# luo-yining/CFDBench

Measured on NVIDIA H100. Metric: fno_rollout_steps_per_sec, higher is better.
Workload: dtype bf16

## Files before the change

cfdbench_b200/csrc/fno_dft_fwd_tc.cu:

```cuda
#include "fno_common.cuh"
#include "tc_common.cuh"
#include "tc_tma.cuh"
#include <math.h>
#include <stddef.h>
#include <string.h>

namespace fno {

constexpr int kTdWG = 2;
constexpr int kTdThreads = 128 * kTdWG;
constexpr int kTdPlanes = 2;
constexpr uint32_t kTdPlaneBytes = kHW * 2;
constexpr uint32_t kTdXBytes = kTdPlanes * kTdPlaneBytes;
constexpr int kTdNA = 72;
constexpr uint32_t kTdLboTA = (kTdNA / 8) * 128;
constexpr uint32_t kTdTABytes = 8 * kTdLboTA;
constexpr int kTdK2 = 128, kTdN2 = kTdPlanes * kM2;
constexpr int kTdM2 = 64;
constexpr uint32_t kTdLboA2 = (kTdM2 / 8) * 128;
constexpr uint32_t kTdLboB2 = (kTdN2 / 8) * 128;
constexpr int kTdA2Floats = kTdM2 * kTdK2;

struct TdSmem {
  alignas(1024) unsigned char x[kTdWG][2][kTdXBytes];
  alignas(128) unsigned char ta[kTdTABytes];
  alignas(128) float a2_hi[kTdA2Floats];
  alignas(128) float a2_lo[kTdA2Floats];
  alignas(128) float b2[kTdWG][2][kTdN2 * kTdK2];
  alignas(8) uint64_t x_full[kTdWG][2];
};

__global__ void __launch_bounds__(kTdThreads, 1)
    dft_fwd_tc_kernel(const __grid_constant__ CUtensorMap x_map, float2* __restrict__ xm,
                      const unsigned char* __restrict__ ta_tab, const float* __restrict__ a2_tab, int n_units, int batch,
                      float s0, float s1) {
  extern __shared__ __align__(1024) unsigned char smem_raw[];
  TdSmem& sm = *reinterpret_cast<TdSmem*>(smem_raw);
  if ((smem_u32(smem_raw) & 1023u) != 0) __trap();
  const int tid = threadIdx.x, lane = tid & 31;
  const int wg = tc::warp_index_uniform() >> 2, wq = (tid >> 5) & 3, t = tid & 127, q = lane & 3;
  const int first = blockIdx.x * kTdWG + wg, stride = gridDim.x * kTdWG;
  const int n_mine = first < n_units ? (n_units - first + stride - 1) / stride : 0;

  if (tid == 0) {
    for (int i = 0; i < kTdWG; ++i) { mbar_init(&sm.x_full[i][0], 1); mbar_init(&sm.x_full[i][1], 1); }
    fence_mbar_init();
  }
  for (int e = tid; e < static_cast<int>(kTdTABytes / 16); e += kTdThreads)
    reinterpret_cast<uint4*>(sm.ta)[e] = __ldg(reinterpret_cast<const uint4*>(ta_tab) + e);
  for (int e = tid; e < kTdA2Floats / 4; e += kTdThreads) {
    reinterpret_cast<float4*>(sm.a2_hi)[e] = __ldg(reinterpret_cast<const float4*>(a2_tab) + e);
    reinterpret_cast<float4*>(sm.a2_lo)[e] = __ldg(reinterpret_cast<const float4*>(a2_tab + kTdA2Floats) + e);
  }
  tc::fence_proxy_async_smem();
  __syncthreads();
  pdl_wait();
  pdl_launch_dependents();

  auto load = [&](int i) {
    mbar_expect_tx(&sm.x_full[wg][i & 1], kTdXBytes);
    tma_load_2d(sm.x[wg][i & 1], &x_map, 0, (first + i * stride) * (kTdPlanes * kH), &sm.x_full[wg][i & 1]);
  };
  if (t == 0) {
    if (n_mine > 0) load(0);
    if (n_mine > 1) load(1);
  }
  const int m0 = 16 * wq + (lane >> 2);
  const uint32_t ta_s = tc::smem_addr(sm.ta);
  float* b2_hi = sm.b2[wg][0];
  float* b2_lo = sm.b2[wg][1];
#pragma unroll 1
  for (int i = 0; i < n_mine; ++i) {
    const int s = i & 1;
    mbar_wait(&sm.x_full[wg][s], (i >> 1) & 1);
    float ga[kTdPlanes][36];
    tc::wg_fence();
    const uint32_t x_s = tc::smem_addr(sm.x[wg][s]);
#pragma unroll
    for (int p = 0; p < kTdPlanes; ++p)
#pragma unroll
      for (int ks = 0; ks < kW / 16; ++ks)
        tc::wg_bf16_ss_n72(ga[p], tc::make_smem_desc_sw128(x_s + p * kTdPlaneBytes + ks * 32),
                           tc::make_smem_desc(ta_s + ks * 2 * kTdLboTA, kTdLboTA, 128), ks ? 1u : 0u);
    tc::wg_commit();
    tc::wg_wait<0>();
    tc::wg_fence_acc(ga[0]);
    tc::wg_fence_acc(ga[1]);
    if (t == 0 && i + 2 < n_mine) load(i + 2);
#pragma unroll
    for (int p = 0; p < kTdPlanes; ++p)
#pragma unroll
      for (int g3 = 0; g3 < 3; ++g3)
#pragma unroll
        for (int hh = 0; hh < 2; ++hh)
#pragma unroll
          for (int ri = 0; ri < 2; ++ri) {
            const int c = 4 * (3 * g3) + 2 * hh + ri;
            const float gsum = (ga[p][c + 8] + ga[p][c + 4]) + ga[p][c];
            float hi, lo;
            tc::split_tf32(gsum, hi, lo);
            const uint32_t off = tc::kmajor_offset(2 * (4 * g3 + q) + p, 64 * ri + m0 + 8 * hh, kTdN2) / 4;
            b2_hi[off] = hi;
            b2_lo[off] = lo;
          }
    tc::fence_proxy_async_smem();
    tc::named_barrier(1 + wg, 128);
    float fb[12];
    tc::wg_fence();
    {
      const uint32_t a_s[3] = {tc::smem_addr(sm.a2_hi), tc::smem_addr(sm.a2_lo), tc::smem_addr(sm.a2_hi)};
      const uint32_t b_s[3] = {tc::smem_addr(b2_hi), tc::smem_addr(b2_hi), tc::smem_addr(b2_lo)};
#pragma unroll
      for (int pass = 0; pass < 3; ++pass)
#pragma unroll
        for (int ks = 0; ks < kTdK2 / 8; ++ks)
          tc::wg_tf32_ss_n24(fb, tc::make_smem_desc(a_s[pass] + ks * 2 * kTdLboA2, kTdLboA2, 128),
                             tc::make_smem_desc(b_s[pass] + ks * 2 * kTdLboB2, kTdLboB2, 128), (pass | ks) ? 1u : 0u);
    }
    tc::wg_commit();
    tc::wg_wait<0>();
    tc::wg_fence_acc(fb);
    const int part = (lane >> 2) & 1;
    const int plane0 = (first + i * stride) * kTdPlanes;
    const int b = plane0 / kC, c0 = plane0 % kC;
#pragma unroll
    for (int j = 0; j < 3; ++j)
#pragma unroll
      for (int hh = 0; hh < 2; ++hh) {
        const int qq = 4 * j + q, m2 = m0 + 8 * hh, kxi = m2 >> 1;
        const float sc = qq == 0 ? s0 : s1;
        const float v0 = fb[4 * j + 2 * hh] * sc, v1 = fb[4 * j + 2 * hh + 1] * sc;
        const float got = __shfl_xor_sync(0xffffffffu, part ? v0 : v1, 4);
        if (m2 < 2 * kKX) {
          float2* dst = xm + (static_cast<size_t>(kxi * kM2 + qq) * batch + b) * kC + c0 + part;
          *dst = part ? make_float2(got, v1) : make_float2(v0, got);
        }
      }
  }
}

static uint16_t td_bf16_bits(double v) {
  float f = static_cast<float>(v);
  uint32_t u;
  memcpy(&u, &f, 4);
  const uint32_t r = u + 0x7fffu + ((u >> 16) & 1u);
  return static_cast<uint16_t>(r >> 16);
}
static double td_bf16_value(uint16_t b) {
  const uint32_t u = static_cast<uint32_t>(b) << 16;
  float f;
  memcpy(&f, &u, 4);
  return static_cast<double>(f);
}
static float td_round_tf32(double v) {
  float f = static_cast<float>(v);
  uint32_t u;
  memcpy(&u, &f, 4);
  u = (u + 0x1000u) & 0xffffe000u;
  memcpy(&f, &u, 4);
  return f;
}

struct TdTables {
  unsigned char* ta = nullptr;
  float* a2 = nullptr;
  int n_sm = 0;
  bool configured = false;
};
static TdTables g_td[64];

static cudaError_t td_ensure(int dev, cudaStream_t stream) {
  TdTables& t = g_td[dev];
  if (t.configured) return cudaSuccess;
  static unsigned char h_ta[kTdTABytes];
  static float h_a2[2 * kTdA2Floats];
  memset(h_ta, 0, sizeof(h_ta));
  memset(h_a2, 0, sizeof(h_a2));
  const double two_pi = 2.0 * 3.14159265358979323846;
  for (int q = 0; q < kM2; ++q)
    for (int ri = 0; ri < 2; ++ri)
      for (int w = 0; w < 64; ++w) {
        const double ang = two_pi * ((q * w) % 64) / 64.0;
        double rest = ri ? -sin(ang) : cos(ang);
        for (int t3 = 0; t3 < 3; ++t3) {
          const int row = 8 * (3 * (q >> 2) + t3) + 2 * (q & 3) + ri;
          const size_t off = static_cast<size_t>(w >> 3) * kTdLboTA + (row >> 3) * 128 + (row & 7) * 16 + (w & 7) * 2;
          const uint16_t bits = td_bf16_bits(rest);
          memcpy(h_ta + off, &bits, 2);
          rest -= td_bf16_value(bits);
        }
      }
  for (int kxi = 0; kxi < kKX; ++kxi) {
    const int kx = kxi < kM1 ? kxi : kxi + (kH - kKX);
    for (int part = 0; part < 2; ++part)
      for (int ri = 0; ri < 2; ++ri)
        for (int h = 0; h < 64; ++h) {
          const double ang = two_pi * ((kx * h) % 64) / 64.0;
          const double c = cos(ang), s = sin(ang);
          const double val = part == 0 ? (ri == 0 ? c : s) : (ri == 0 ? -s : c);
          const uint32_t off = tc::kmajor_offset(2 * kxi + part, ri * 64 + h, kTdM2) / 4;
          const float hi = td_round_tf32(val);
          h_a2[off] = hi;
          h_a2[kTdA2Floats + off] = td_round_tf32(val - static_cast<double>(hi));
        }
  }
  cudaError_t e = cudaMalloc(&t.ta, sizeof(h_ta));
  if (e != cudaSuccess) return e;
  e = cudaMalloc(&t.a2, sizeof(h_a2));
  if (e != cudaSuccess) return e;
  e = cudaMemcpyAsync(t.ta, h_ta, sizeof(h_ta), cudaMemcpyHostToDevice, stream);
  if (e != cudaSuccess) return e;
  e = cudaMemcpyAsync(t.a2, h_a2, sizeof(h_a2), cudaMemcpyHostToDevice, stream);
  if (e != cudaSuccess) return e;
  e = cudaStreamSynchronize(stream);
  if (e != cudaSuccess) return e;
  e = cudaFuncSetAttribute(dft_fwd_tc_kernel, cudaFuncAttributeMaxDynamicSharedMemorySize, (int)sizeof(TdSmem));
  if (e != cudaSuccess) return e;
  e = cudaDeviceGetAttribute(&t.n_sm, cudaDevAttrMultiProcessorCount, dev);
  if (e != cudaSuccess) return e;
  t.configured = true;
  return cudaSuccess;
}

void dft_fwd_tc_release(int dev) {
  if (dev < 0 || dev >= 64) return;
  TdTables& t = g_td[dev];
  if (t.ta) cudaFree(t.ta);
  if (t.a2) cudaFree(t.a2);
  t = TdTables();
}

cudaError_t launch_dft_fwd_tc(const void* x, void* xm, int batch, float s0, float s1, cudaStream_t stream) {
  int dev = 0;
  cudaError_t e = cudaGetDevice(&dev);
  if (e != cudaSuccess) return e;
  if (dev < 0 || dev >= 64) return cudaErrorInvalidDevice;
  e = td_ensure(dev, stream);
  if (e != cudaSuccess) return e;
  if ((reinterpret_cast<uintptr_t>(x) & 15) || (reinterpret_cast<uintptr_t>(xm) & 15)) return cudaErrorMisalignedAddress;
  CUtensorMap map;
  e = make_tma_map_2d(&map, CU_TENSOR_MAP_DATA_TYPE_BFLOAT16, 2, x, kW, static_cast<uint64_t>(batch) * kC * kH, kW,
                      kTdPlanes * kH);
  if (e != cudaSuccess) return e;
  const int n_units = batch * kC / kTdPlanes;
  const int want = (n_units + kTdWG - 1) / kTdWG;
  const int grid = want < g_td[dev].n_sm ? want : g_td[dev].n_sm;
  return launch_chained(dft_fwd_tc_kernel, dim3(grid), dim3(kTdThreads), sizeof(TdSmem), stream, map,
                        static_cast<float2*>(xm), static_cast<const unsigned char*>(g_td[dev].ta),
                        static_cast<const float*>(g_td[dev].a2), n_units, batch, s0, s1);
}

}
```

cfdbench_b200/csrc/tc_common.cuh:

```cuda
#pragma once
#include <cuda_runtime.h>
#include <stdint.h>

namespace fno {
namespace tc {

__device__ __forceinline__ uint32_t smem_addr(const void* p) {
  return static_cast<uint32_t>(__cvta_generic_to_shared(p));
}

__device__ __forceinline__ int warp_index_uniform() {
  return __shfl_sync(0xffffffffu, static_cast<int>(threadIdx.x >> 5), 0);
}

__device__ __forceinline__ void named_barrier(int id, int count) {
  asm volatile("bar.sync %0, %1;" ::"r"(id), "r"(count) : "memory");
}

__device__ __forceinline__ void fence_proxy_async_smem() {
  asm volatile("fence.proxy.async.shared::cta;" ::: "memory");
}

__device__ __forceinline__ uint64_t make_smem_desc(uint32_t saddr, uint32_t lbo_bytes, uint32_t sbo_bytes) {
  uint64_t d = 0;
  d |= static_cast<uint64_t>((saddr & 0x3FFFFu) >> 4);
  d |= static_cast<uint64_t>((lbo_bytes >> 4) & 0x3FFFu) << 16;
  d |= static_cast<uint64_t>((sbo_bytes >> 4) & 0x3FFFu) << 32;
  return d;
}
__device__ __forceinline__ uint64_t make_smem_desc_sw128(uint32_t saddr) {
  return make_smem_desc(saddr, 16, 1024) | (static_cast<uint64_t>(1) << 62);
}
__device__ __forceinline__ uint64_t make_smem_desc_sw128_mn(uint32_t saddr) {
  return make_smem_desc(saddr, 16, 1024) | (static_cast<uint64_t>(1) << 62);
}

__device__ __forceinline__ void wg_fence() { asm volatile("wgmma.fence.sync.aligned;" ::: "memory"); }
__device__ __forceinline__ void wg_commit() { asm volatile("wgmma.commit_group.sync.aligned;" ::: "memory"); }
template <int kPending>
__device__ __forceinline__ void wg_wait() { asm volatile("wgmma.wait_group.sync.aligned %0;" ::"n"(kPending) : "memory"); }
template <int N>
__device__ __forceinline__ void wg_fence_acc(float (&d)[N]) {
#pragma unroll
  for (int i = 0; i < N; ++i) asm volatile("" : "+f"(d[i])::"memory");
}

__device__ __forceinline__ void wg_tf32_ss_n24(float* d, uint64_t a, uint64_t b, uint32_t acc) {
  asm volatile(
      "{\n.reg .pred p;\nsetp.ne.b32 p, %14, 0;\n"
      "wgmma.mma_async.sync.aligned.m64n24k8.f32.tf32.tf32 {%0, %1, %2, %3, %4, %5, %6, %7, %8, %9, %10, %11}, %12, %13, p, 1, 1;\n}\n"
      : "+f"(d[0]), "+f"(d[1]), "+f"(d[2]), "+f"(d[3]), "+f"(d[4]), "+f"(d[5]), "+f"(d[6]), "+f"(d[7]), "+f"(d[8]), "+f"(d[9]), "+f"(d[10]), "+f"(d[11])
      : "l"(a), "l"(b), "r"(acc)
      : "memory");
}
__device__ __forceinline__ void wg_tf32_ss_n32(float* d, uint64_t a, uint64_t b, uint32_t acc) {
  asm volatile(
      "{\n.reg .pred p;\nsetp.ne.b32 p, %18, 0;\n"
      "wgmma.mma_async.sync.aligned.m64n32k8.f32.tf32.tf32 {%0, %1, %2, %3, %4, %5, %6, %7, %8, %9, %10, %11, %12, %13, %14, %15}, %16, %17, p, 1, 1;\n}\n"
      : "+f"(d[0]), "+f"(d[1]), "+f"(d[2]), "+f"(d[3]), "+f"(d[4]), "+f"(d[5]), "+f"(d[6]), "+f"(d[7]), "+f"(d[8]), "+f"(d[9]), "+f"(d[10]), "+f"(d[11]), "+f"(d[12]), "+f"(d[13]), "+f"(d[14]), "+f"(d[15])
      : "l"(a), "l"(b), "r"(acc)
      : "memory");
}
__device__ __forceinline__ void wg_tf32_ss_n128(float* d, uint64_t a, uint64_t b, uint32_t acc) {
  asm volatile(
      "{\n.reg .pred p;\nsetp.ne.b32 p, %66, 0;\n"
      "wgmma.mma_async.sync.aligned.m64n128k8.f32.tf32.tf32 {%0, %1, %2, %3, %4, %5, %6, %7, %8, %9, %10, %11, %12, %13, %14, %15, %16, %17, %18, %19, %20, %21, %22, %23, %24, %25, %26, %27, %28, %29, %30, %31, %32, %33, %34, %35, %36, %37, %38, %39, %40, %41, %42, %43, %44, %45, %46, %47, %48, %49, %50, %51, %52, %53, %54, %55, %56, %57, %58, %59, %60, %61, %62, %63}, %64, %65, p, 1, 1;\n}\n"
      : "+f"(d[0]), "+f"(d[1]), "+f"(d[2]), "+f"(d[3]), "+f"(d[4]), "+f"(d[5]), "+f"(d[6]), "+f"(d[7]), "+f"(d[8]), "+f"(d[9]), "+f"(d[10]), "+f"(d[11]), "+f"(d[12]), "+f"(d[13]), "+f"(d[14]), "+f"(d[15]), "+f"(d[16]), "+f"(d[17]), "+f"(d[18]), "+f"(d[19]), "+f"(d[20]), "+f"(d[21]), "+f"(d[22]), "+f"(d[23]), "+f"(d[24]), "+f"(d[25]), "+f"(d[26]), "+f"(d[27]), "+f"(d[28]), "+f"(d[29]), "+f"(d[30]), "+f"(d[31]), "+f"(d[32]), "+f"(d[33]), "+f"(d[34]), "+f"(d[35]), "+f"(d[36]), "+f"(d[37]), "+f"(d[38]), "+f"(d[39]), "+f"(d[40]), "+f"(d[41]), "+f"(d[42]), "+f"(d[43]), "+f"(d[44]), "+f"(d[45]), "+f"(d[46]), "+f"(d[47]), "+f"(d[48]), "+f"(d[49]), "+f"(d[50]), "+f"(d[51]), "+f"(d[52]), "+f"(d[53]), "+f"(d[54]), "+f"(d[55]), "+f"(d[56]), "+f"(d[57]), "+f"(d[58]), "+f"(d[59]), "+f"(d[60]), "+f"(d[61]), "+f"(d[62]), "+f"(d[63])
      : "l"(a), "l"(b), "r"(acc)
      : "memory");
}
__device__ __forceinline__ void wg_bf16_ss_n72(float* d, uint64_t a, uint64_t b, uint32_t acc) {
  asm volatile(
      "{\n.reg .pred p;\nsetp.ne.b32 p, %38, 0;\n"
      "wgmma.mma_async.sync.aligned.m64n72k16.f32.bf16.bf16 {%0, %1, %2, %3, %4, %5, %6, %7, %8, %9, %10, %11, %12, %13, %14, %15, %16, %17, %18, %19, %20, %21, %22, %23, %24, %25, %26, %27, %28, %29, %30, %31, %32, %33, %34, %35}, %36, %37, p, 1, 1, 0, 0;\n}\n"
      : "+f"(d[0]), "+f"(d[1]), "+f"(d[2]), "+f"(d[3]), "+f"(d[4]), "+f"(d[5]), "+f"(d[6]), "+f"(d[7]), "+f"(d[8]), "+f"(d[9]), "+f"(d[10]), "+f"(d[11]), "+f"(d[12]), "+f"(d[13]), "+f"(d[14]), "+f"(d[15]), "+f"(d[16]), "+f"(d[17]), "+f"(d[18]), "+f"(d[19]), "+f"(d[20]), "+f"(d[21]), "+f"(d[22]), "+f"(d[23]), "+f"(d[24]), "+f"(d[25]), "+f"(d[26]), "+f"(d[27]), "+f"(d[28]), "+f"(d[29]), "+f"(d[30]), "+f"(d[31]), "+f"(d[32]), "+f"(d[33]), "+f"(d[34]), "+f"(d[35])
      : "l"(a), "l"(b), "r"(acc)
      : "memory");
}
__device__ __forceinline__ void wg_bf16_ss_n32_mn_a(float* d, uint64_t a, uint64_t b, uint32_t acc) {
  asm volatile(
      "{\n.reg .pred p;\nsetp.ne.b32 p, %18, 0;\n"
      "wgmma.mma_async.sync.aligned.m64n32k16.f32.bf16.bf16 {%0, %1, %2, %3, %4, %5, %6, %7, %8, %9, %10, %11, %12, %13, %14, %15}, %16, %17, p, 1, 1, 1, 0;\n}\n"
      : "+f"(d[0]), "+f"(d[1]), "+f"(d[2]), "+f"(d[3]), "+f"(d[4]), "+f"(d[5]), "+f"(d[6]), "+f"(d[7]), "+f"(d[8]), "+f"(d[9]), "+f"(d[10]), "+f"(d[11]), "+f"(d[12]), "+f"(d[13]), "+f"(d[14]), "+f"(d[15])
      : "l"(a), "l"(b), "r"(acc)
      : "memory");
}
__device__ __forceinline__ void wg_tf32_rs_n32(float* d, const uint32_t* a, uint64_t b, uint32_t acc) {
  asm volatile(
      "{\n.reg .pred p;\nsetp.ne.b32 p, %21, 0;\n"
      "wgmma.mma_async.sync.aligned.m64n32k8.f32.tf32.tf32 {%0, %1, %2, %3, %4, %5, %6, %7, %8, %9, %10, %11, %12, %13, %14, %15}, {%16, %17, %18, %19}, %20, p, 1, 1;\n}\n"
      : "+f"(d[0]), "+f"(d[1]), "+f"(d[2]), "+f"(d[3]), "+f"(d[4]), "+f"(d[5]), "+f"(d[6]), "+f"(d[7]), "+f"(d[8]), "+f"(d[9]), "+f"(d[10]), "+f"(d[11]), "+f"(d[12]), "+f"(d[13]), "+f"(d[14]), "+f"(d[15])
      : "r"(a[0]), "r"(a[1]), "r"(a[2]), "r"(a[3]), "l"(b), "r"(acc)
      : "memory");
}
__device__ __forceinline__ void wg_tf32_rs_n64(float* d, const uint32_t* a, uint64_t b, uint32_t acc) {
  asm volatile(
      "{\n.reg .pred p;\nsetp.ne.b32 p, %37, 0;\n"
      "wgmma.mma_async.sync.aligned.m64n64k8.f32.tf32.tf32 {%0, %1, %2, %3, %4, %5, %6, %7, %8, %9, %10, %11, %12, %13, %14, %15, %16, %17, %18, %19, %20, %21, %22, %23, %24, %25, %26, %27, %28, %29, %30, %31}, {%32, %33, %34, %35}, %36, p, 1, 1;\n}\n"
      : "+f"(d[0]), "+f"(d[1]), "+f"(d[2]), "+f"(d[3]), "+f"(d[4]), "+f"(d[5]), "+f"(d[6]), "+f"(d[7]), "+f"(d[8]), "+f"(d[9]), "+f"(d[10]), "+f"(d[11]), "+f"(d[12]), "+f"(d[13]), "+f"(d[14]), "+f"(d[15]), "+f"(d[16]), "+f"(d[17]), "+f"(d[18]), "+f"(d[19]), "+f"(d[20]), "+f"(d[21]), "+f"(d[22]), "+f"(d[23]), "+f"(d[24]), "+f"(d[25]), "+f"(d[26]), "+f"(d[27]), "+f"(d[28]), "+f"(d[29]), "+f"(d[30]), "+f"(d[31])
      : "r"(a[0]), "r"(a[1]), "r"(a[2]), "r"(a[3]), "l"(b), "r"(acc)
      : "memory");
}

__host__ __device__ constexpr uint32_t kmajor_offset(int row, int k, int rows) {
  return static_cast<uint32_t>(((k >> 2) * (rows >> 3) + (row >> 3)) * 128 + (row & 7) * 16 + (k & 3) * 4);
}
__device__ __forceinline__ float round_tf32(float x) {
  return __uint_as_float((__float_as_uint(x) + 0x1000u) & 0xffffe000u);
}
__device__ __forceinline__ void split_tf32(float x, float& hi, float& lo) {
  hi = round_tf32(x);
  lo = round_tf32(x - hi);
}

}
}
```

Baseline: 1202.

## Restructure forward DFT stage B to batch eight planes per unit with register-A TF32 wgmma

Each work unit grows from two to eight planes, loaded as four two-plane TMA boxes through a three-slot pipeline. The second (H-direction) DFT stage is transposed so the plane/mode dimension becomes M (three full m64 tiles) and the twiddle table becomes the shared-memory B operand. Intermediates are staged in a swizzled fp32 buffer and split into hi/lo TF32 in registers for RS wgmma at n48. This is meant to replace the narrow n24 stage-B MMAs, which were padded and under-used, with fuller tiles, and to cut the shuffle-based output writes. In exchange it needs more shared memory, more registers per thread for the A fragments, and a grid sized to balance units per pipe.

```diff
diff --git a/cfdbench_b200/csrc/fno_dft_fwd_tc.cu b/cfdbench_b200/csrc/fno_dft_fwd_tc.cu
--- a/cfdbench_b200/csrc/fno_dft_fwd_tc.cu
+++ b/cfdbench_b200/csrc/fno_dft_fwd_tc.cu
@@ -9,133 +9,153 @@
 
 constexpr int kTdWG = 2;
 constexpr int kTdThreads = 128 * kTdWG;
-constexpr int kTdPlanes = 2;
+constexpr int kTdPlanes = 8;
+constexpr int kTdBoxPlanes = 2;
+constexpr int kTdBoxes = kTdPlanes / kTdBoxPlanes;
+constexpr int kTdSlots = 3;
 constexpr uint32_t kTdPlaneBytes = kHW * 2;
-constexpr uint32_t kTdXBytes = kTdPlanes * kTdPlaneBytes;
+constexpr uint32_t kTdBoxBytes = kTdBoxPlanes * kTdPlaneBytes;
 constexpr int kTdNA = 72;
 constexpr uint32_t kTdLboTA = (kTdNA / 8) * 128;
 constexpr uint32_t kTdTABytes = 8 * kTdLboTA;
-constexpr int kTdK2 = 128, kTdN2 = kTdPlanes * kM2;
-constexpr int kTdM2 = 64;
-constexpr uint32_t kTdLboA2 = (kTdM2 / 8) * 128;
-constexpr uint32_t kTdLboB2 = (kTdN2 / 8) * 128;
-constexpr int kTdA2Floats = kTdM2 * kTdK2;
+constexpr int kTdM2 = kM2 * 2 * kTdPlanes;
+constexpr int kTdN2 = 2 * kKX;
+constexpr int kTdK2 = kH;
+constexpr uint32_t kTdLboT = (kTdN2 / 8) * 128;
+constexpr int kTdTFloats = kTdN2 * kTdK2;
+static_assert(kTdM2 == 3 * 64, "stage B is three full m64 tiles");
+
+__host__ __device__ constexpr int td_slot(int n) { return n % kTdSlots; }
+__host__ __device__ constexpr uint32_t td_parity(int n) { return static_cast<uint32_t>(n / kTdSlots) & 1u; }
+__host__ __device__ constexpr int td_box_row(int unit, int box) { return (unit * kTdPlanes + box * kTdBoxPlanes) * kH; }
+__host__ __device__ constexpr int td_unit(int first, int stride, int i) { return first + i * stride; }
+__host__ __device__ constexpr int td_units_of(int first, int stride, int n_units) {
+  return first < n_units ? (n_units - first + stride - 1) / stride : 0;
+}
+__host__ __device__ constexpr int td_g_index(int m, int h) {
+  return m * kTdK2 + (h ^ (((m & 7) << 2) ^ (((m >> 4) & 3) << 3)));
+}
 
 struct TdSmem {
-  alignas(1024) unsigned char x[kTdWG][2][kTdXBytes];
+  alignas(1024) unsigned char x[kTdWG][kTdSlots][kTdBoxBytes];
   alignas(128) unsigned char ta[kTdTABytes];
-  alignas(128) float a2_hi[kTdA2Floats];
-  alignas(128) float a2_lo[kTdA2Floats];
-  alignas(128) float b2[kTdWG][2][kTdN2 * kTdK2];
-  alignas(8) uint64_t x_full[kTdWG][2];
+  alignas(128) float t_hi[kTdTFloats];
+  alignas(128) float t_lo[kTdTFloats];
+  alignas(128) float g[kTdWG][kTdM2 * kTdK2];
+  alignas(8) uint64_t x_full[kTdWG][kTdSlots];
 };
+static_assert(sizeof(TdSmem) <= 232448, "dft_fwd_tc_kernel exceeds the sm_90 opt-in shared memory");
 
 __global__ void __launch_bounds__(kTdThreads, 1)
     dft_fwd_tc_kernel(const __grid_constant__ CUtensorMap x_map, float2* __restrict__ xm,
-                      const unsigned char* __restrict__ ta_tab, const float* __restrict__ a2_tab, int n_units, int batch,
+                      const unsigned char* __restrict__ ta_tab, const float* __restrict__ t_tab, int n_units, int batch,
                       float s0, float s1) {
   extern __shared__ __align__(1024) unsigned char smem_raw[];
   TdSmem& sm = *reinterpret_cast<TdSmem*>(smem_raw);
   if ((smem_u32(smem_raw) & 1023u) != 0) __trap();
   const int tid = threadIdx.x, lane = tid & 31;
-  const int wg = tc::warp_index_uniform() >> 2, wq = (tid >> 5) & 3, t = tid & 127, q = lane & 3;
+  const int wg = tc::warp_index_uniform() >> 2, wq = (tid >> 5) & 3, t = tid & 127, q = lane & 3, lr = lane >> 2;
   const int first = blockIdx.x * kTdWG + wg, stride = gridDim.x * kTdWG;
-  const int n_mine = first < n_units ? (n_units - first + stride - 1) / stride : 0;
+  const int n_mine = td_units_of(first, stride, n_units);
+  const int n_fills = n_mine * kTdBoxes;
 
   if (tid == 0) {
-    for (int i = 0; i < kTdWG; ++i) { mbar_init(&sm.x_full[i][0], 1); mbar_init(&sm.x_full[i][1], 1); }
+    for (int i = 0; i < kTdWG; ++i)
+      for (int s = 0; s < kTdSlots; ++s) mbar_init(&sm.x_full[i][s], 1);
     fence_mbar_init();
   }
   for (int e = tid; e < static_cast<int>(kTdTABytes / 16); e += kTdThreads)
     reinterpret_cast<uint4*>(sm.ta)[e] = __ldg(reinterpret_cast<const uint4*>(ta_tab) + e);
-  for (int e = tid; e < kTdA2Floats / 4; e += kTdThreads) {
-    reinterpret_cast<float4*>(sm.a2_hi)[e] = __ldg(reinterpret_cast<const float4*>(a2_tab) + e);
-    reinterpret_cast<float4*>(sm.a2_lo)[e] = __ldg(reinterpret_cast<const float4*>(a2_tab + kTdA2Floats) + e);
+  for (int e = tid; e < kTdTFloats / 4; e += kTdThreads) {
+    reinterpret_cast<float4*>(sm.t_hi)[e] = __ldg(reinterpret_cast<const float4*>(t_tab) + e);
+    reinterpret_cast<float4*>(sm.t_lo)[e] = __ldg(reinterpret_cast<const float4*>(t_tab + kTdTFloats) + e);
   }
   tc::fence_proxy_async_smem();
   __syncthreads();
   pdl_wait();
   pdl_launch_dependents();
 
-  auto load = [&](int i) {
-    mbar_expect_tx(&sm.x_full[wg][i & 1], kTdXBytes);
-    tma_load_2d(sm.x[wg][i & 1], &x_map, 0, (first + i * stride) * (kTdPlanes * kH), &sm.x_full[wg][i & 1]);
+  auto load = [&](int n) {
+    uint64_t* bar = &sm.x_full[wg][td_slot(n)];
+    mbar_expect_tx(bar, kTdBoxBytes);
+    tma_load_2d(sm.x[wg][td_slot(n)], &x_map, 0, td_box_row(td_unit(first, stride, n / kTdBoxes), n % kTdBoxes), bar);
   };
-  if (t == 0) {
-    if (n_mine > 0) load(0);
-    if (n_mine > 1) load(1);
-  }
-  const int m0 = 16 * wq + (lane >> 2);
+  if (t == 0)
+    for (int n = 0; n < kTdSlots && n < n_fills; ++n) load(n);
+  const int m0 = 16 * wq + lr;
   const uint32_t ta_s = tc::smem_addr(sm.ta);
-  float* b2_hi = sm.b2[wg][0];
-  float* b2_lo = sm.b2[wg][1];
+  float* g = sm.g[wg];
 #pragma unroll 1
   for (int i = 0; i < n_mine; ++i) {
-    const int s = i & 1;
-    mbar_wait(&sm.x_full[wg][s], (i >> 1) & 1);
-    float ga[kTdPlanes][36];
-    tc::wg_fence();
-    const uint32_t x_s = tc::smem_addr(sm.x[wg][s]);
-#pragma unroll
-    for (int p = 0; p < kTdPlanes; ++p)
-#pragma unroll
-      for (int ks = 0; ks < kW / 16; ++ks)
-        tc::wg_bf16_ss_n72(ga[p], tc::make_smem_desc_sw128(x_s + p * kTdPlaneBytes + ks * 32),
-                           tc::make_smem_desc(ta_s + ks * 2 * kTdLboTA, kTdLboTA, 128), ks ? 1u : 0u);
-    tc::wg_commit();
-    tc::wg_wait<0>();
-    tc::wg_fence_acc(ga[0]);
-    tc::wg_fence_acc(ga[1]);
-    if (t == 0 && i + 2 < n_mine) load(i + 2);
-#pragma unroll
-    for (int p = 0; p < kTdPlanes; ++p)
-#pragma unroll
-      for (int g3 = 0; g3 < 3; ++g3)
-#pragma unroll
-        for (int hh = 0; hh < 2; ++hh)
-#pragma unroll
-          for (int ri = 0; ri < 2; ++ri) {
-            const int c = 4 * (3 * g3) + 2 * hh + ri;
-            const float gsum = (ga[p][c + 8] + ga[p][c + 4]) + ga[p][c];
-            float hi, lo;
-            tc::split_tf32(gsum, hi, lo);
-            const uint32_t off = tc::kmajor_offset(2 * (4 * g3 + q) + p, 64 * ri + m0 + 8 * hh, kTdN2) / 4;
-            b2_hi[off] = hi;
-            b2_lo[off] = lo;
-          }
-    tc::fence_proxy_async_smem();
+#pragma unroll 1
+    for (int k = 0; k < kTdBoxes; ++k) {
+      const int n = i * kTdBoxes + k;
+      mbar_wait(&sm.x_full[wg][td_slot(n)], td_parity(n));
+      float ga[kTdBoxPlanes][36];
+      tc::wg_fence();
+      const uint32_t x_s = tc::smem_addr(sm.x[wg][td_slot(n)]);
+#pragma unroll
+      for (int p = 0; p < kTdBoxPlanes; ++p)
+#pragma unroll
+        for (int ks = 0; ks < kW / 16; ++ks)
+          tc::wg_bf16_ss_n72(ga[p], tc::make_smem_desc_sw128(x_s + p * kTdPlaneBytes + ks * 32),
+                             tc::make_smem_desc(ta_s + ks * 2 * kTdLboTA, kTdLboTA, 128), ks ? 1u : 0u);
+      tc::wg_commit();
+      tc::wg_wait<0>();
+      tc::wg_fence_acc(ga[0]);
+      tc::wg_fence_acc(ga[1]);
+      if (t == 0 && n + kTdSlots < n_fills) load(n + kTdSlots);
+      if (k == 0) tc::named_barrier(1 + wg, 128);
+#pragma unroll
+      for (int p = 0; p < kTdBoxPlanes; ++p)
+#pragma unroll
+        for (int g3 = 0; g3 < 3; ++g3)
+#pragma unroll
+          for (int hh = 0; hh < 2; ++hh)
+#pragma unroll
+            for (int ri = 0; ri < 2; ++ri) {
+              const int c = 4 * (3 * g3) + 2 * hh + ri;
+              g[td_g_index(16 * (4 * g3 + q) + 8 * ri + kTdBoxPlanes * k + p, m0 + 8 * hh)] =
+                  (ga[p][c + 8] + ga[p][c + 4]) + ga[p][c];
+            }
+    }
     tc::named_barrier(1 + wg, 128);
-    float fb[12];
-    tc::wg_fence();
-    {
-      const uint32_t a_s[3] = {tc::smem_addr(sm.a2_hi), tc::smem_addr(sm.a2_lo), tc::smem_addr(sm.a2_hi)};
-      const uint32_t b_s[3] = {tc::smem_addr(b2_hi), tc::smem_addr(b2_hi), tc::smem_addr(b2_lo)};
-#pragma unroll
-      for (int pass = 0; pass < 3; ++pass)
+    const int unit = td_unit(first, stride, i);
+    const int b = unit * kTdPlanes / kC, c0 = unit * kTdPlanes % kC;
+#pragma unroll 1
+    for (int tile = 0; tile < kTdM2 / 64; ++tile) {
+      uint32_t a_hi[kTdK2 / 8][4], a_lo[kTdK2 / 8][4];
+#pragma unroll
+      for (int ks = 0; ks < kTdK2 / 8; ++ks)
+#pragma unroll
+        for (int r = 0; r < 4; ++r) {
+          float hi, lo;
+          tc::split_tf32(g[td_g_index(64 * tile + m0 + 8 * (r & 1), 8 * ks + q + 4 * (r >> 1))], hi, lo);
+          a_hi[ks][r] = __float_as_uint(hi);
+          a_lo[ks][r] = __float_as_uint(lo);
+        }
+      float d[24];
+      tc::wg_fence();
+#pragma unroll
+      for (int pass = 0; pass < 3; ++pass) {
+        const uint32_t tb = tc::smem_addr(pass == 1 ? sm.t_lo : sm.t_hi);
 #pragma unroll
         for (int ks = 0; ks < kTdK2 / 8; ++ks)
-          tc::wg_tf32_ss_n24(fb, tc::make_smem_desc(a_s[pass] + ks * 2 * kTdLboA2, kTdLboA2, 128),
-                             tc::make_smem_desc(b_s[pass] + ks * 2 * kTdLboB2, kTdLboB2, 128), (pass | ks) ? 1u : 0u);
+          tc::wg_tf32_rs_n48(d, pass == 2 ? a_lo[ks] : a_hi[ks], tc::make_smem_desc(tb + ks * 2 * kTdLboT, kTdLboT, 128),
+                             (pass | ks) ? 1u : 0u);
+      }
+      tc::wg_commit();
+      tc::wg_wait<0>();
+      tc::wg_fence_acc(d);
+      const int qq = 4 * tile + wq;
+      const float sc = qq == 0 ? s0 : s1;
+#pragma unroll
+      for (int j = 0; j < kTdN2 / 8; ++j) {
+        const int kxi = 4 * j + q;
+        const float re = (d[4 * j + 0] + d[4 * j + 3]) * sc, im = (d[4 * j + 2] - d[4 * j + 1]) * sc;
+        xm[(static_cast<size_t>(kxi * kM2 + qq) * batch + b) * kC + c0 + lr] = make_float2(re, im);
+      }
     }
-    tc::wg_commit();
-    tc::wg_wait<0>();
-    tc::wg_fence_acc(fb);
-    const int part = (lane >> 2) & 1;
-    const int plane0 = (first + i * stride) * kTdPlanes;
-    const int b = plane0 / kC, c0 = plane0 % kC;
-#pragma unroll
-    for (int j = 0; j < 3; ++j)
-#pragma unroll
-      for (int hh = 0; hh < 2; ++hh) {
-        const int qq = 4 * j + q, m2 = m0 + 8 * hh, kxi = m2 >> 1;
-        const float sc = qq == 0 ? s0 : s1;
-        const float v0 = fb[4 * j + 2 * hh] * sc, v1 = fb[4 * j + 2 * hh + 1] * sc;
-        const float got = __shfl_xor_sync(0xffffffffu, part ? v0 : v1, 4);
-        if (m2 < 2 * kKX) {
-          float2* dst = xm + (static_cast<size_t>(kxi * kM2 + qq) * batch + b) * kC + c0 + part;
-          *dst = part ? make_float2(got, v1) : make_float2(v0, got);
-        }
-      }
   }
 }
 
@@ -163,7 +183,7 @@
 
 struct TdTables {
   unsigned char* ta = nullptr;
-  float* a2 = nullptr;
+  float* t = nullptr;
   int n_sm = 0;
   bool configured = false;
 };
@@ -173,9 +193,9 @@
   TdTables& t = g_td[dev];
   if (t.configured) return cudaSuccess;
   static unsigned char h_ta[kTdTABytes];
-  static float h_a2[2 * kTdA2Floats];
+  static float h_t[2 * kTdTFloats];
   memset(h_ta, 0, sizeof(h_ta));
-  memset(h_a2, 0, sizeof(h_a2));
+  memset(h_t, 0, sizeof(h_t));
   const double two_pi = 2.0 * 3.14159265358979323846;
   for (int q = 0; q < kM2; ++q)
     for (int ri = 0; ri < 2; ++ri)
@@ -192,25 +212,23 @@
       }
   for (int kxi = 0; kxi < kKX; ++kxi) {
     const int kx = kxi < kM1 ? kxi : kxi + (kH - kKX);
-    for (int part = 0; part < 2; ++part)
-      for (int ri = 0; ri < 2; ++ri)
-        for (int h = 0; h < 64; ++h) {
-          const double ang = two_pi * ((kx * h) % 64) / 64.0;
-          const double c = cos(ang), s = sin(ang);
-          const double val = part == 0 ? (ri == 0 ? c : s) : (ri == 0 ? -s : c);
-          const uint32_t off = tc::kmajor_offset(2 * kxi + part, ri * 64 + h, kTdM2) / 4;
-          const float hi = td_round_tf32(val);
-          h_a2[off] = hi;
-          h_a2[kTdA2Floats + off] = td_round_tf32(val - static_cast<double>(hi));
-        }
+    for (int cs = 0; cs < 2; ++cs)
+      for (int h = 0; h < kH; ++h) {
+        const double ang = two_pi * ((kx * h) % 64) / 64.0;
+        const double val = cs ? sin(ang) : cos(ang);
+        const uint32_t off = tc::kmajor_offset(2 * kxi + cs, h, kTdN2) / 4;
+        const float hi = td_round_tf32(val);
+        h_t[off] = hi;
+        h_t[kTdTFloats + off] = td_round_tf32(val - static_cast<double>(hi));
+      }
   }
   cudaError_t e = cudaMalloc(&t.ta, sizeof(h_ta));
   if (e != cudaSuccess) return e;
-  e = cudaMalloc(&t.a2, sizeof(h_a2));
+  e = cudaMalloc(&t.t, sizeof(h_t));
   if (e != cudaSuccess) return e;
   e = cudaMemcpyAsync(t.ta, h_ta, sizeof(h_ta), cudaMemcpyHostToDevice, stream);
   if (e != cudaSuccess) return e;
-  e = cudaMemcpyAsync(t.a2, h_a2, sizeof(h_a2), cudaMemcpyHostToDevice, stream);
+  e = cudaMemcpyAsync(t.t, h_t, sizeof(h_t), cudaMemcpyHostToDevice, stream);
   if (e != cudaSuccess) return e;
   e = cudaStreamSynchronize(stream);
   if (e != cudaSuccess) return e;
@@ -226,7 +244,7 @@
   if (dev < 0 || dev >= 64) return;
   TdTables& t = g_td[dev];
   if (t.ta) cudaFree(t.ta);
-  if (t.a2) cudaFree(t.a2);
+  if (t.t) cudaFree(t.t);
   t = TdTables();
 }
 
@@ -240,14 +258,14 @@
   if ((reinterpret_cast<uintptr_t>(x) & 15) || (reinterpret_cast<uintptr_t>(xm) & 15)) return cudaErrorMisalignedAddress;
   CUtensorMap map;
   e = make_tma_map_2d(&map, CU_TENSOR_MAP_DATA_TYPE_BFLOAT16, 2, x, kW, static_cast<uint64_t>(batch) * kC * kH, kW,
-                      kTdPlanes * kH);
+                      kTdBoxPlanes * kH);
   if (e != cudaSuccess) return e;
   const int n_units = batch * kC / kTdPlanes;
-  const int want = (n_units + kTdWG - 1) / kTdWG;
-  const int grid = want < g_td[dev].n_sm ? want : g_td[dev].n_sm;
+  const int per_pipe = (n_units + kTdWG * g_td[dev].n_sm - 1) / (kTdWG * g_td[dev].n_sm);
+  const int grid = (n_units + kTdWG * per_pipe - 1) / (kTdWG * per_pipe);
   return launch_chained(dft_fwd_tc_kernel, dim3(grid), dim3(kTdThreads), sizeof(TdSmem), stream, map,
                         static_cast<float2*>(xm), static_cast<const unsigned char*>(g_td[dev].ta),
-                        static_cast<const float*>(g_td[dev].a2), n_units, batch, s0, s1);
-}
-
-}
+                        static_cast<const float*>(g_td[dev].t), n_units, batch, s0, s1);
+}
+
+}
diff --git a/cfdbench_b200/csrc/tc_common.cuh b/cfdbench_b200/csrc/tc_common.cuh
--- a/cfdbench_b200/csrc/tc_common.cuh
+++ b/cfdbench_b200/csrc/tc_common.cuh
@@ -45,14 +45,6 @@
   for (int i = 0; i < N; ++i) asm volatile("" : "+f"(d[i])::"memory");
 }
 
-__device__ __forceinline__ void wg_tf32_ss_n24(float* d, uint64_t a, uint64_t b, uint32_t acc) {
-  asm volatile(
-      "{\n.reg .pred p;\nsetp.ne.b32 p, %14, 0;\n"
-      "wgmma.mma_async.sync.aligned.m64n24k8.f32.tf32.tf32 {%0, %1, %2, %3, %4, %5, %6, %7, %8, %9, %10, %11}, %12, %13, p, 1, 1;\n}\n"
-      : "+f"(d[0]), "+f"(d[1]), "+f"(d[2]), "+f"(d[3]), "+f"(d[4]), "+f"(d[5]), "+f"(d[6]), "+f"(d[7]), "+f"(d[8]), "+f"(d[9]), "+f"(d[10]), "+f"(d[11])
-      : "l"(a), "l"(b), "r"(acc)
-      : "memory");
-}
 __device__ __forceinline__ void wg_tf32_ss_n32(float* d, uint64_t a, uint64_t b, uint32_t acc) {
   asm volatile(
       "{\n.reg .pred p;\nsetp.ne.b32 p, %18, 0;\n"
@@ -93,6 +85,14 @@
       : "r"(a[0]), "r"(a[1]), "r"(a[2]), "r"(a[3]), "l"(b), "r"(acc)
       : "memory");
 }
+__device__ __forceinline__ void wg_tf32_rs_n48(float* d, const uint32_t* a, uint64_t b, uint32_t acc) {
+  asm volatile(
+      "{\n.reg .pred p;\nsetp.ne.b32 p, %29, 0;\n"
+      "wgmma.mma_async.sync.aligned.m64n48k8.f32.tf32.tf32 {%0, %1, %2, %3, %4, %5, %6, %7, %8, %9, %10, %11, %12, %13, %14, %15, %16, %17, %18, %19, %20, %21, %22, %23}, {%24, %25, %26, %27}, %28, p, 1, 1;\n}\n"
+      : "+f"(d[0]), "+f"(d[1]), "+f"(d[2]), "+f"(d[3]), "+f"(d[4]), "+f"(d[5]), "+f"(d[6]), "+f"(d[7]), "+f"(d[8]), "+f"(d[9]), "+f"(d[10]), "+f"(d[11]), "+f"(d[12]), "+f"(d[13]), "+f"(d[14]), "+f"(d[15]), "+f"(d[16]), "+f"(d[17]), "+f"(d[18]), "+f"(d[19]), "+f"(d[20]), "+f"(d[21]), "+f"(d[22]), "+f"(d[23])
+      : "r"(a[0]), "r"(a[1]), "r"(a[2]), "r"(a[3]), "l"(b), "r"(acc)
+      : "memory");
+}
 __device__ __forceinline__ void wg_tf32_rs_n64(float* d, const uint32_t* a, uint64_t b, uint32_t acc) {
   asm volatile(
       "{\n.reg .pred p;\nsetp.ne.b32 p, %37, 0;\n"
```

Result: faster. 1277 (median of 6 runs) (+6.3%).
